# oooolga/Ctrl-V

Hardware: AMD Instinct MI355X
Metric: denoising steps/sec, SVD+ControlNet 25f 576x1024 (higher is better)
Workload: dtype bf16; 1 GPU; box2video: ControlNet + UNet forward, CFG batch 2, 25 frames, latent 72x128, 25-step Karras Euler schedule, random-init SVD-XT weights; clips_per_gpu=1, parallelism=clip-shard x1, hip_graph=True

## Files before the change

### ctrlv_amd/_lib.py

```python
import ctypes
import os
import threading

_HERE = os.path.dirname(os.path.abspath(__file__))
LIB_PATH = os.path.join(_HERE, "lib", "libctrlv_hip.so")
LIB_PATH_F16 = os.path.join(_HERE, "lib", "libctrlv_hip_f16.so")

c_void_p, c_int, c_float, c_size_t = ctypes.c_void_p, ctypes.c_int32, ctypes.c_float, ctypes.c_size_t


class GemmDesc(ctypes.Structure):
    _fields_ = [
        ("A", c_void_p), ("A2", c_void_p), ("W", c_void_p), ("out", c_void_p),
        ("bias", c_void_p), ("R1", c_void_p), ("R2", c_void_p), ("V", c_void_p),
        ("M", c_int), ("N", c_int), ("Cin", c_int), ("taps", c_int),
        ("lda", c_int), ("lda2", c_int), ("c_split", c_int),
        ("mode", c_int),
        ("H", c_int), ("Wd", c_int), ("Ho", c_int), ("Wo", c_int), ("stride", c_int), ("up", c_int),
        ("F", c_int), ("S", c_int),
        ("ldo", c_int), ("n_store", c_int),
        ("ldr1", c_int), ("ldr2", c_int),
        ("s_acc", c_float), ("s1", c_float), ("s2", c_float),
        ("vmode", c_int), ("vdiv", c_int), ("vmod", c_int), ("vS", c_int), ("ldv", c_int),
        ("act", c_int), ("geglu", c_int), ("out_f32", c_int), ("tile", c_int),
# ... 85 lines not shown
        ("latents", c_void_p), ("sigmas", ctypes.POINTER(c_float)), ("timesteps", ctypes.POINTER(c_float)),
        ("fps", c_int), ("motion_bucket_id", c_int),
        ("min_guidance", c_float), ("max_guidance", c_float), ("conditioning_scale", c_float), ("decode_chunk", c_int),
        ("clip_mean", c_float * 3), ("clip_std", c_float * 3),
        ("out_latents", c_void_p), ("out_frames", c_void_p), ("out_frames_u8", c_void_p),
    ]


SIGNATURES = {
    "ctrlv_abi_version": (c_int, []),
    "ctrlv_elem_dtype": (c_int, []),
    "ctrlv_build_id": (c_int, [ctypes.c_char_p, c_size_t]),
    "ctrlv_last_error": (c_int, [ctypes.c_char_p, c_size_t]),
    "ctrlv_gemm": (c_int, [ctypes.POINTER(GemmDesc), c_void_p]),
    "ctrlv_gemm_gn_partials_serves": (c_int, [ctypes.POINTER(GemmDesc)]),
    "ctrlv_gemm_splitk_ws_bytes": (c_size_t, [ctypes.POINTER(GemmDesc)]),
    "ctrlv_gemm_up_phase_serves": (c_int, [ctypes.POINTER(GemmDesc)]),
    "ctrlv_pack_up_phase_weight": (c_int, [c_void_p, c_int, c_int, c_int, c_void_p, c_void_p]),
    "ctrlv_groupnorm_from_partials": (c_int, [c_void_p, c_int, c_int, c_int, c_int, c_float, c_void_p, c_void_p, c_void_p,
                                              c_int, c_void_p, c_void_p]),
    "ctrlv_groupnorm_from_partials_split": (c_int, [c_void_p, c_void_p, c_int, c_int, c_int, c_int, c_float, c_void_p, c_void_p, c_void_p,
                                              c_int, c_void_p, c_void_p]),
    "ctrlv_groupnorm_chunks": (c_int, [c_int, c_int, c_int, c_int]),
    "ctrlv_groupnorm_stats_split": (c_int, [c_void_p, c_void_p, c_void_p, c_void_p, c_int, c_int, c_int, c_int, c_int, c_float,
                                            c_void_p, c_void_p]),
    "ctrlv_groupnorm_apply_split": (c_int, [c_void_p, c_void_p, c_void_p, c_void_p, c_int, c_int, c_int, c_int, c_int, c_void_p,
                                            c_void_p, c_void_p, c_int, c_void_p, c_void_p]),
    "ctrlv_layernorm_split": (c_int, [c_void_p, c_void_p, c_int, c_int, c_void_p, c_void_p, c_float, c_void_p, c_int, c_int,
                                      c_int, c_void_p, c_void_p]),
    "ctrlv_axpby_split": (c_int, [c_void_p, c_void_p, c_void_p, c_float, c_float, c_void_p, c_void_p, c_size_t, c_void_p]),
    "ctrlv_plan_set_trunk_mode": (c_int, [c_void_p, c_int]),
    "ctrlv_plan_set_ff_precision": (c_int, [c_void_p, c_int]),
    "ctrlv_groupnorm_stats": (c_int, [c_void_p, c_void_p, c_int, c_int, c_int, c_int, c_int, c_float, c_void_p,
                                      c_void_p]),
    "ctrlv_groupnorm_apply": (c_int, [c_void_p, c_void_p, c_int, c_int, c_int, c_int, c_int, c_void_p, c_void_p,
                                      c_void_p, c_int, c_void_p, c_void_p]),
    "ctrlv_layernorm": (c_int, [c_void_p, c_int, c_int, c_void_p, c_void_p, c_float, c_void_p, c_int, c_int, c_int,
                                c_void_p, c_void_p]),
    "ctrlv_softmax_rows": (c_int, [c_void_p, c_int, c_int, ctypes.c_long, c_void_p, ctypes.c_long, c_void_p]),
    "ctrlv_softmax_rows_bwd": (c_int, [c_void_p, ctypes.c_long, c_void_p, ctypes.c_long, c_int, c_int, c_float, c_void_p,
                                       ctypes.c_long, c_void_p]),
    "ctrlv_ff_fused_w1f_bytes": (c_int, []),
    "ctrlv_ff_fused_pack": (c_int, [c_void_p, c_void_p, c_void_p, c_void_p, c_void_p, c_void_p]),
    "ctrlv_ff_fused_serves": (c_int, [ctypes.POINTER(GemmDesc), c_int]),
    "ctrlv_ff_fused": (c_int, [c_void_p, c_int, c_void_p, c_void_p, ctypes.POINTER(GemmDesc), c_void_p]),
    "ctrlv_ff_fused_ln": (c_int, [c_void_p, c_int, c_void_p, c_void_p, c_float, c_void_p, c_int, c_int, c_int, c_void_p,
# ... 210 lines not shown
```

### ctrlv_amd/csrc/abi.hip

```cpp
#include <stdarg.h>
#include <stdlib.h>

#include <mutex>

#include "common.h"

#ifndef CTRLV_BUILD_ID
#define CTRLV_BUILD_ID "unstamped"
#endif

static thread_local char g_err[512] = "";
void ctrlv_set_error(const char* fmt, ...) {
  va_list ap;
  va_start(ap, fmt);
  vsnprintf(g_err, sizeof(g_err), fmt, ap);
  va_end(ap);
}

const ctrlv_debug_t& ctrlv_debug() {
  static const ctrlv_debug_t dbg = [] {
    auto env = [](const char* name, int dflt) { const char* e = getenv(name); return e ? atoi(e) : dflt; };
    ctrlv_debug_t d;
    d.w16 = env("CTRLV_W16", 1);
    d.splitk = env("CTRLV_SPLITK", 1);
    d.force_tile = env("CTRLV_GEMM_FORCE_TILE", 0);
    d.conv_halo = env("CTRLV_CONV_HALO", 1);
    d.gn_fused = env("CTRLV_GN_FUSED", 1);
    d.gn_cross = env("CTRLV_GN_CROSS", 1);
    d.gn_rev = env("CTRLV_GN_REV", 1);
    d.gn_rows = env("CTRLV_GN_ROWS", 256);
    if (d.gn_rows < 32 || d.gn_rows > 1024) d.gn_rows = 256;
    d.ln_rows = env("CTRLV_LN_ROWS", 1);
    d.ff_fused = env("CTRLV_FF_FUSED", 1);
    d.ff_ln = env("CTRLV_FF_LN", 0);
    d.pp_balanced = env("CTRLV_PP_BALANCED", 1);
    d.pp_cgrp = env("CTRLV_PP_CGRP", 0);
    d.attn_rows = env("CTRLV_ATTN_ROWS", 0);
    d.temporal_fused = env("CTRLV_TEMPORAL_FUSED", 1);
    d.wgrad_pp = env("CTRLV_WGRAD_PP", 1);
    d.wgrad_slabs = env("CTRLV_WGRAD_SLABS", 0);
    d.up_phase = env("CTRLV_UP_PHASE", 1);
    return d;
  }();
  return dbg;
}

int ctrlv_current_device() {
  int dev = 0;
  if (hipGetDevice(&dev) != hipSuccess || dev < 0 || dev >= CTRLV_MAX_DEVICES) dev = 0;
  return dev;
}

int ctrlv_num_cu(int dev) {
  static int cu[CTRLV_MAX_DEVICES] = {};
  static std::mutex mu;
// ... 33 lines not shown
```

### ctrlv_amd/csrc/common.h

```cpp
#pragma once
#include <hip/hip_runtime.h>
#include <stdint.h>
#include <stdio.h>
#include <string.h>

#include "../../include/ctrlv_hip.h"

#ifdef CTRLV_ELEM_F16
typedef _Float16 el_native_t;
#define CTRLV_ELEM_DTYPE 1
#define CTRLV_MFMA_32x32x16_ASM "v_mfma_f32_32x32x16_f16"
#else
typedef __bf16 el_native_t;
#define CTRLV_ELEM_DTYPE 2
#define CTRLV_MFMA_32x32x16_ASM "v_mfma_f32_32x32x16_bf16"
#endif
typedef __attribute__((ext_vector_type(8))) el_native_t elx8;
typedef __attribute__((ext_vector_type(4))) el_native_t elx4;
typedef __attribute__((ext_vector_type(2))) el_native_t elx2;
typedef __attribute__((ext_vector_type(16))) float f32x16;
typedef __attribute__((ext_vector_type(4))) float f32x4;
typedef __attribute__((ext_vector_type(4))) short s16x4;
typedef uint16_t el_t;
typedef uint16_t bf16_t;
// ... 227 lines not shown
  extern "C" int ctrlv_debug_clock_##unit(unsigned long long* out2, int reset) {                                   \
    if (hipDeviceSynchronize() != hipSuccess) return -3;                                                           \
    if (out2 && hipMemcpyFromSymbol(out2, HIP_SYMBOL(g_ctrlv_clock), 16) != hipSuccess) return -3;                 \
    const unsigned long long z[2] = {0, 0};                                                                        \
    if (reset && hipMemcpyToSymbol(HIP_SYMBOL(g_ctrlv_clock), z, 16) != hipSuccess) return -3;                     \
    return 0;                                                                                                      \
  }
#else
#define CTRLV_CLOCK_BEGIN()
#define CTRLV_CLOCK_END()
#define CTRLV_CLOCK_READER(unit)
#endif

struct ctrlv_debug_t {
  int w16;
  int splitk;
  int force_tile;
  int conv_halo;
  int gn_fused;
  int gn_cross;
  int gn_rev;
  int gn_rows;
  int ln_rows;
  int ff_fused;
  int ff_ln;
  int pp_balanced;
  int pp_cgrp;
  int attn_rows;
  int temporal_fused;
  int wgrad_pp;
  int wgrad_slabs;
  int up_phase;
};
const ctrlv_debug_t& ctrlv_debug();
void ctrlv_set_error(const char* fmt, ...);
#define CTRLV_MAX_DEVICES 64
int ctrlv_current_device();
int ctrlv_num_cu(int dev);
size_t ctrlv_gemm_tokens_counter_bytes(int M, int N, int K);
const ctrlv_model_config* ctrlv_plan_info(const ctrlv_plan* p, int* device, int* loaded);
const ctrlv_clip_config* ctrlv_clip_plan_info(const ctrlv_clip_plan* p, int* device, int* loaded);
const ctrlv_vae_config* ctrlv_vae_plan_info(const ctrlv_vae_plan* p, int* device, int* loaded);
#define CTRLV_CHECK_ARG(cond, ...)                  \
  do {                                              \
    if (!(cond)) {                                  \
      ctrlv_set_error(__VA_ARGS__);                 \
// ... 39 lines not shown
```

### ctrlv_amd/csrc/norm.hip

```cpp
#include <stdlib.h>

#include "common.h"

namespace {

struct GnShape {
  int n_img, S, C, imgs_per_stat, c_split, n_chunks, rows_per_chunk, CV, RPP;
  int rev_stats, rev_apply;
};

__device__ __forceinline__ uint4 gn_load(const el_t* x, const el_t* x2, int c_split, int C, long row, int c0) {
  if (x2 != nullptr && c0 >= c_split) return *(const uint4*)(x2 + row * (C - c_split) + (c0 - c_split));
  const int ld = x2 != nullptr ? c_split : C;
  return *(const uint4*)(x + row * ld + c0);
}
struct GnLo { const lo_t* x; const lo_t* x2; };
__device__ __forceinline__ const lo_t* gn_lo_plane(const GnLo& lo, const el_t* x2, int c_split, int C, int c0, int* ld, int* first) {
  if (x2 != nullptr && c0 >= c_split) { *ld = C - c_split; *first = c_split; return lo.x2; }
  *ld = x2 != nullptr ? c_split : C; *first = 0;
  return lo.x;
}

template <bool SPLIT>
__global__ void gn_stats_kernel(const el_t* __restrict__ x, const el_t* __restrict__ x2, GnLo lo, GnShape s,
// ... 158 lines not shown
  for (; r < r1; r += s.RPP) apply_row(gn_load(x, x2, s.c_split, s.C, (long)n * s.S + r, c0), (long)n * s.S + r);
}

int gn_shape(int n_img, int S, int C, int imgs_per_stat, int c_split, bool has_x2, GnShape* s) {
  CTRLV_CHECK_SHAPE(n_img > 0 && S > 0 && C > 0 && C % 32 == 0 && C % 8 == 0 && C <= 8192,
                    "groupnorm: C=%d must be a multiple of 32 (and of 8), <= 8192", C);
  CTRLV_CHECK_SHAPE(imgs_per_stat > 0 && n_img % imgs_per_stat == 0, "groupnorm: n_img %% imgs_per_stat != 0");
  if (has_x2) CTRLV_CHECK_SHAPE(c_split > 0 && c_split < C && c_split % 8 == 0, "groupnorm: bad c_split %d", c_split);
  s->n_img = n_img; s->S = S; s->C = C; s->imgs_per_stat = imgs_per_stat; s->c_split = c_split;
  s->CV = C / 8;
  s->RPP = s->CV >= 256 ? 1 : 256 / s->CV;
  {
    const int rev = ctrlv_debug().gn_rev;
    s->rev_stats = rev & 1; s->rev_apply = (rev >> 1) & 1;
  }
  {
    const int rpc_big = ctrlv_debug().gn_rows;
    s->rows_per_chunk = S >= 4096 ? rpc_big : (S >= 1024 ? 64 : 32);
  }
  if ((S + s->rows_per_chunk - 1) / s->rows_per_chunk > 256) s->rows_per_chunk = (((S + 255) / 256) + 255) / 256 * 256;
  if (s->rows_per_chunk > S) s->rows_per_chunk = S;
  s->n_chunks = (S + s->rows_per_chunk - 1) / s->rows_per_chunk;
  return CTRLV_OK;
}

template <int NV>
__global__ __launch_bounds__(256) void ln_kernel(const el_t* __restrict__ x, const lo_t* __restrict__ xlo, int M, int C,
                                                 const float* __restrict__ gamma, const float* __restrict__ beta,
                                                 float eps, const float* __restrict__ V, int vdiv, int vmod, int ldv,
                                                 el_t* __restrict__ y) {
  const int lane = threadIdx.x & 63, wid = threadIdx.x >> 6;
  const int CV = C >> 3;
  float g[NV][8], b[NV][8];
#pragma unroll
  for (int k = 0; k < NV; ++k) {
    const int cv = lane + k * 64;
    if (cv < CV) {
#pragma unroll
      for (int e = 0; e < 8; ++e) { g[k][e] = gamma[cv * 8 + e]; b[k][e] = beta[cv * 8 + e]; }
    }
  }
  const float inv_c = 1.0f / (float)C;
  const long step = (long)gridDim.x * 4;
  long m = (long)blockIdx.x * 4 + wid;
  uint4 nxt[NV];
#pragma unroll
// ... 297 lines not shown
  CTRLV_CHECK_ARG(x && partials && gamma && beta && y, "groupnorm_from_partials: null pointer");
  CTRLV_CHECK_SHAPE(S > 0 && S % 64 == 0, "groupnorm_from_partials: S=%d must be a multiple of 64", S);
  GnShape s;
  int rc = gn_shape(n_img, S, C, imgs_per_stat, 0, false, &s);
  if (rc < 0) return rc;
  GnShape sp = s;
  sp.rows_per_chunk = 64;
  sp.n_chunks = S / 64;
  float* stats = partials + (size_t)n_img * sp.n_chunks * 64;
  hipLaunchKernelGGL(gn_finalize_kernel, dim3(n_img / imgs_per_stat, 32 / kFinGroups), dim3(1024), 0, (hipStream_t)stream, sp,
                     partials, eps, stats);
  CTRLV_LAUNCH_CHECK();
  const int nt = s.CV * s.RPP;
  if (x_lo)
    hipLaunchKernelGGL(gn_apply_kernel<true>, dim3(s.n_chunks, n_img), dim3(nt), 0, (hipStream_t)stream, (const el_t*)x,
                       (const el_t*)nullptr, GnLo{(const lo_t*)x_lo, nullptr}, s, stats, gamma, beta, silu, (el_t*)y);
  else
    hipLaunchKernelGGL(gn_apply_kernel<false>, dim3(s.n_chunks, n_img), dim3(nt), 0, (hipStream_t)stream, (const el_t*)x,
                       (const el_t*)nullptr, GnLo{nullptr, nullptr}, s, stats, gamma, beta, silu, (el_t*)y);
  CTRLV_LAUNCH_CHECK();
  return CTRLV_OK;
}

extern "C" int ctrlv_layernorm(const void* x, int M, int C, const float* gamma, const float* beta, float eps,
                               const float* V, int vdiv, int vmod, int ldv, void* y, ctrlv_stream_t stream) {
  return ctrlv_layernorm_split(x, nullptr, M, C, gamma, beta, eps, V, vdiv, vmod, ldv, y, stream);
}
extern "C" int ctrlv_layernorm_split(const void* x, const void* x_lo, int M, int C, const float* gamma, const float* beta,
                                     float eps, const float* V, int vdiv, int vmod, int ldv, void* y, ctrlv_stream_t stream) {
  CTRLV_CHECK_ARG(x && gamma && beta && y, "layernorm: null pointer");
  CTRLV_CHECK_SHAPE(M > 0 && C > 0 && C % 8 == 0 && C <= 2048, "layernorm: C=%d must be a multiple of 8, <= 2048", C);
  if (V) CTRLV_CHECK_ARG(vdiv > 0 && vmod > 0 && ldv >= C, "layernorm: bad row-vector table");
  const int nv = (C / 8 + 63) / 64;
  hipStream_t st = (hipStream_t)stream;
  const int rows_path = ctrlv_debug().ln_rows;
  const int lpr = C / 40;
  if (rows_path && C % 40 == 0 && (lpr == 8 || lpr == 16 || lpr == 32) && (!V || (ldv % 4 == 0 && ((uintptr_t)V & 15) == 0))) {
    const int lg = lpr == 8 ? 3 : (lpr == 16 ? 4 : 5), rpb = 4 * (64 >> lg);
    long nb = ((long)M + rpb - 1) / rpb;
    if (nb > 256 * 8) nb = 256 * 8;
    if (x_lo)
      hipLaunchKernelGGL((ln_rows_kernel<5, true>), dim3((unsigned)nb), dim3(256), 2 * C * sizeof(float), st, (const el_t*)x,
                         (const lo_t*)x_lo, M, C, lg, gamma, beta, eps, V, vdiv, vmod, ldv, (el_t*)y);
    else
      hipLaunchKernelGGL((ln_rows_kernel<5, false>), dim3((unsigned)nb), dim3(256), 2 * C * sizeof(float), st, (const el_t*)x,
                         (const lo_t*)nullptr, M, C, lg, gamma, beta, eps, V, vdiv, vmod, ldv, (el_t*)y);
// ... 19 lines not shown
```

### ctrlv_amd/csrc/plan.hip

```cpp
#include <math.h>

#include <string>
#include <vector>

#include "weight_loader.h"

namespace {

using ctrlv_load::WeightLoader;
using Linear = ctrlv_load::PackedLinear;
using Norm = ctrlv_load::NormParams;

__global__ void arange_kernel(float* dst, int n) {
  const int i = blockIdx.x * blockDim.x + threadIdx.x;
  if (i < n) dst[i] = (float)i;
}
__global__ void expand_f32_kernel(const float* __restrict__ src, int n_src, float* __restrict__ dst, int n) {
  const int i = blockIdx.x * blockDim.x + threadIdx.x;
  if (i < n) dst[i] = src[n_src == 1 ? 0 : i];
}

struct ResBlock {
  int cin = 0, cout = 0;
  float eps = 1e-6f;
// ... 294 lines not shown
           (d.R1 ? (double)d.M * n_out * 2 : 0) + (d.R2 ? (double)d.M * n_out * 2 : 0) +
           ((d.R1_lo ? 1 : 0) + (d.R2_lo ? 1 : 0) + (d.out_lo ? 1 : 0)) * (double)d.M * n_out;
}
inline void set_r1(ctrlv_gemm_desc& d, const Trk& t, int ld) { d.R1 = t.hi; d.R1_lo = t.lo; d.ldr1 = ld; }
inline void set_r2(ctrlv_gemm_desc& d, const Trk& t, int ld) { d.R2 = t.hi; d.R2_lo = t.lo; d.ldr2 = ld; }
inline void set_out(ctrlv_gemm_desc& d, const Trk& t) { d.out = t.hi; d.out_lo = t.lo; }

int gemm(Ctx& c, const ctrlv_gemm_desc& d0) {
  ctrlv_gemm_desc d = d0;
  const size_t mk = c.mark();
  const size_t ws = ctrlv_gemm_splitk_ws_bytes(&d);
  if (ws) d.splitk_ws = c.alloc(ws);
  int rc = CTRLV_OK;
  if (!c.dry) {
    if (c.overflow) { ctrlv_set_error("plan forward: workspace too small (need >= %zu bytes)", c.peak); return CTRLV_E_BAD_ARG; }
    int fam; double fl, by;
    gemm_work(d, &fam, &fl, &by);
    ProfScope ps(c, fam, fl, by, d.M, d.N, (d.mode == 1 && d.up == 2 ? 4 : d.taps) * d.Cin, (d.geglu ? 1 : 0) | ((d.R1 ? 1 : 0) + (d.R2 ? 1 : 0)) << 1 | d.vmode << 3);
    rc = ctrlv_gemm(&d, c.st);
  }
  c.release(mk);
  return rc;
}
int groupnorm(Ctx& c, const Trk& x, const Trk& x2, int c_split, int n_img, int S, int C, int ips, const Norm& nm,
              float eps, int silu, el_t* y) {
  const int chunks = ctrlv_groupnorm_chunks(n_img, S, C, ips);
  if (chunks < 0) return chunks;
  const size_t m = c.mark();
  float* part = (float*)c.alloc(((size_t)n_img * chunks + n_img / ips) * 64 * 4);
  int rc = CTRLV_OK;
  if (!c.dry) {
    if (c.overflow) { ctrlv_set_error("plan forward: workspace too small (need >= %zu bytes)", c.peak); return CTRLV_E_BAD_ARG; }
    ProfScope ps(c, CTRLV_FAM_GROUPNORM, 0.0, 2.0 * 2 * n_img * (double)S * C, n_img * S, C);
    rc = ctrlv_groupnorm_stats_split(x.hi, x.lo, x2.hi, x2.lo, c_split, n_img, S, C, ips, eps, part, c.st);
    if (rc == CTRLV_OK)
      rc = ctrlv_groupnorm_apply_split(x.hi, x.lo, x2.hi, x2.lo, c_split, n_img, S, C, ips, part, nm.g, nm.b, silu, y, c.st);
  }
  c.release(m);
  return rc;
}
int gemm_groupnorm(Ctx& c, ctrlv_gemm_desc d, int n_img, int S, int C, int ips, const Norm& nm, float eps, int silu, el_t* y) {
  const Trk dout{(el_t*)d.out, (lo_t*)d.out_lo};
  if (S % 64 != 0) {
    CTRLV_TRY(gemm(c, d));
    return groupnorm(c, dout, Trk{}, 0, n_img, S, C, ips, nm, eps, silu, y);
  }
  const size_t m = c.mark();
  float* part = (float*)c.alloc(((size_t)n_img * (S / 64) + n_img / ips) * 64 * 4);
  int rc = CTRLV_OK;
  if (!c.dry && ctrlv_gemm_gn_partials_serves(&d)) {
    d.gn_partials = part;
    rc = gemm(c, d);
    if (rc == CTRLV_OK) {
      ProfScope ps(c, CTRLV_FAM_GROUPNORM, 0.0, 2.0 * 2 * n_img * (double)S * C, n_img * S, C, 1);
      rc = ctrlv_groupnorm_from_partials_split(d.out, d.out_lo, n_img, S, C, ips, eps, part, nm.g, nm.b, silu, y, c.st);
    }
// ... 887 lines not shown
```

### ctrlv_amd/models/blocks.py

```python
import math
import os

import torch
from torch import nn

from .. import ops, packing
from ..lora import merged_weight


class FwdCtx:

    def __init__(self, ws, B, F, temb, xattn, time_context_order):
        self.ws, self.B, self.F = ws, B, F
        self.temb = temb
        self.xattn = xattn
        self.quirk = time_context_order == "sb"
        self.gn_part = None
        self.gn_cross = None
        self.gn_cross_valid = False
        self.trace = None


def _sigmoid(x):
    return 1.0 / (1.0 + math.exp(-x))
# ... 153 lines not shown


def _ln_ff(ws, xraw, ln, t, ffp, ubox, out, C, ln_V=None, ln_vdiv=1, ln_vmod=1 << 30, rows_per_image=0, **epi):
    if _FF_FUSED and _FF_LN and len(ffp) == 6 and _lo(xraw) is None and ops.ff_fused_serves(xraw, out, **_trk_epi(epi, out)):
        ops.ff_fused(xraw, ffp[4], ffp[5], out, bias=ffp[3], ln=(ln[0], ln[1], 1e-5), ln_V=ln_V, ln_vdiv=ln_vdiv,
                     ln_vmod=ln_vmod, **_trk_epi(epi, out))
        return
    if getattr(ws, "ff_f8", False) and _lo(xraw) is None and _ff_f8_route(ws, xraw, ln, ffp, ubox, out, C, ln_V, ln_vdiv, ln_vmod, epi):
        return
    if ln_V is not None:
        ops.layernorm(xraw, ln[0], ln[1], 1e-5, t, V=ln_V, vdiv=ln_vdiv, vmod=ln_vmod, x_lo=_lo(xraw))
    else:
        ops.layernorm(xraw, ln[0], ln[1], 1e-5, t, x_lo=_lo(xraw))
    _ff_pair(ws, t, ffp, ubox, out, C, rows_per_image=rows_per_image, **epi)


def _gn_scratch(ctx, n_img, S, C, ips):
    need = ops.groupnorm_scratch_floats(n_img, S, C, ips)
    if ctx.gn_part is None or ctx.gn_part.numel() < need:
        ctx.gn_part = torch.empty(max(need, 1 << 18), dtype=torch.float32, device=ctx.ws.device)
    return ctx.gn_part


def _gemm_groupnorm(ctx, A, W, out, gkw, n_img, S, C, ips, gamma, beta, eps, y):
    gkw = _trk_epi(gkw, out)
    if S % 64 == 0 and ops.gemm_gn_partials_serves(A, W, out, **gkw):
        need = ops.groupnorm_fused_scratch_floats(n_img, S, ips)
        if ctx.gn_part is None or ctx.gn_part.numel() < need:
            ctx.gn_part = torch.empty(max(need, 1 << 18), dtype=torch.float32, device=ctx.ws.device)
        ops.gemm(A, W, out, gn_partials=ctx.gn_part, **gkw)
        ops.groupnorm_from_partials(out, n_img, S, C, ips, gamma, beta, eps, True, y, ctx.gn_part, x_lo=_lo(out))
    else:
        ops.gemm(A, W, out, **gkw)
        ops.groupnorm(out, None, n_img, S, C, ips, gamma, beta, eps, True, y, _gn_scratch(ctx, n_img, S, C, ips),
                      x_lo=_lo(out))


class SpatioTemporalResBlock(nn.Module):
    def __init__(self, in_channels, out_channels, temb_channels, eps=1e-6):
        super().__init__()
        self.cin, self.cout, self.eps = in_channels, out_channels, eps
        self.spatial_res_block = _ResnetBlock2D(in_channels, out_channels, temb_channels, eps)
        self.temporal_res_block = _TemporalResnetBlock(out_channels, temb_channels, eps)
        self.time_mixer = _AlphaBlender(0.5)
        self.temb_off = None
        self._pk = None

    def temb_projections(self):
        return [self.spatial_res_block.time_emb_proj, self.temporal_res_block.time_emb_proj]

    def pack(self):
        s, t = self.spatial_res_block, self.temporal_res_block
        pk = dict(
            g1=_f32(s.norm1.weight), b1=_f32(s.norm1.bias), w1=packing.pack_conv3x3(s.conv1.weight),
            cb1=_f32(s.conv1.bias),
            g2=_f32(s.norm2.weight), b2=_f32(s.norm2.bias), w2=packing.pack_conv3x3(s.conv2.weight),
            cb2=_f32(s.conv2.bias),
            tg1=_f32(t.norm1.weight), tb1=_f32(t.norm1.bias), tw1=packing.pack_conv_temporal(t.conv1.weight),
            tcb1=_f32(t.conv1.bias),
            tg2=_f32(t.norm2.weight), tb2=_f32(t.norm2.bias), tw2=packing.pack_conv_temporal(t.conv2.weight),
            tcb2=_f32(t.conv2.bias),
            alpha=_sigmoid(float(self.time_mixer.mix_factor.detach().float().cpu())),
        )
        if s.conv_shortcut is not None:
            pk["wsc"] = packing.pack_linear(s.conv_shortcut.weight)
            pk["bsc"] = _f32(s.conv_shortcut.bias)
        self._pk = pk

    def run(self, ctx, x, H, W, x2=None, feeds_norm=False):
        pk, ws = self._pk, ctx.ws
        B, F = ctx.B, ctx.F
        N, S = B * F, H * W
        M = N * S
        cin, cout = self.cin, self.cout
        out = ws.trunk((M, cout))
        mk = ws.mark()
        part = _gn_scratch(ctx, N, S, max(cin, cout), 1)
        xn = ws.alloc((M, cin))
        ops.groupnorm(x, x2, N, S, cin, 1, pk["g1"], pk["b1"], self.eps, True, xn, part, x_lo=_lo(x), x2_lo=_lo(x2))
        h = ws.alloc((M, cout))
        vs = ctx.temb[:, self.temb_off[0]:]
        hn = ws.alloc((M, cout))
        _gemm_groupnorm(ctx, xn, pk["w1"], h, dict(N=cout, cin=cin, taps=9, mode=1, conv=(H, W, H, W, 1, 0), bias=pk["cb1"],
                                                   V=vs, vmode=1, vdiv=F * S),
                        N, S, cout, 1, pk["g2"], pk["b2"], self.eps, hn)
        if "wsc" in pk:
            res = ws.trunk((M, cout))
            ops.gemm(x, pk["wsc"], res, N=cout, cin=cin, A2=x2, c_split=x.shape[1] if x2 is not None else 0,
                     bias=pk["bsc"], out_lo=_lo(res))
        else:
            res = x
        xs = ws.trunk((M, cout))
        _gemm_groupnorm(ctx, hn, pk["w2"], xs, dict(N=cout, cin=cout, taps=9, mode=1, conv=(H, W, H, W, 1, 0), bias=pk["cb2"],
                                                    R1=res),
                        N, S, cout, F, pk["tg1"], pk["tb1"], self.eps, hn)
        vt = ctx.temb[:, self.temb_off[1]:]
        _gemm_groupnorm(ctx, hn, pk["tw1"], h, dict(N=cout, cin=cout, taps=3, mode=2, temporal=(F, S), bias=pk["tcb1"],
                                                    V=vt, vmode=1, vdiv=F * S),
                        N, S, cout, F, pk["tg2"], pk["tb2"], self.eps, hn)
        kw2 = _trk_epi(dict(N=cout, cin=cout, taps=3, mode=2, temporal=(F, S), bias=pk["tcb2"], s_acc=1.0 - pk["alpha"], R1=xs),
                       out)
        ctx.gn_cross_valid = False
# ... 79 lines not shown
            kp = pk["tpe"][0].shape[1]
            te = torch.zeros(F, kp, dtype=el, device=device)
            if kp == C:
                ops.timestep_embedding(t, C, te)
            else:
                tmp = torch.empty(F, C, dtype=el, device=device)
                ops.timestep_embedding(t, C, tmp)
                te[:, :C] = tmp
            h = torch.empty(F, 4 * C, dtype=el, device=device)
            ops.gemm(te, pk["tpe"][0], h, N=4 * C, cin=kp, bias=pk["tpe"][1], act=1)
            e = torch.empty(F, C, dtype=torch.float32, device=device)
            ops.gemm(h, pk["tpe"][2], e, N=C, cin=4 * C, bias=pk["tpe"][3], out_f32=True)
            self._frame_emb[F] = e
        return self._frame_emb[F]

    def run(self, ctx, x, H, W):
        pk, ws = self._pk, ctx.ws
        B, F, C = ctx.B, ctx.F, self.C
        N, S = B * F, H * W
        M = N * S
        emb = self.frame_embedding(F, x.device)
        out = ws.trunk((M, C))
        mk = ws.mark()
        part = _gn_scratch(ctx, N, S, C, 1)
        t = ws.alloc((M, C))
        if ctx.gn_cross_valid:
            ctx.gn_cross_valid = False
            ops.groupnorm_from_partials(x, N, S, C, 1, pk["gn"][0], pk["gn"][1], 1e-6, False, t, ctx.gn_cross, x_lo=_lo(x))
        else:
            ops.groupnorm(x, None, N, S, C, 1, pk["gn"][0], pk["gn"][1], 1e-6, False, t, part, x_lo=_lo(x))
        h0 = ws.trunk((M, C))
        ops.gemm(t, pk["pin"][0], h0, N=C, cin=C, bias=pk["pin"][1], out_lo=_lo(h0))
        ops.layernorm(h0, pk["s_ln1"][0], pk["s_ln1"][1], 1e-5, t, x_lo=_lo(h0))
        qkv = ws.alloc((M, 3 * C))
        ops.gemm(t, pk["s_qkv"], qkv, N=3 * C, cin=C, n_scale2=C, s_acc2=ops.Q_PRESCALE)
        a = ws.alloc((M, C))
        ops.attention_spatial(qkv, a, N, S, C, prescaled=True)
        h1 = ws.trunk((M, C))
        xs_vec = ctx.xattn[:, self.xattn_off[0]:]
        ops.gemm(a, pk["s_o"][0], h1, N=C, cin=C, bias=pk["s_o"][1], **_trk_epi(dict(R1=h0, V=xs_vec, vmode=1, vdiv=F * S), h1))
        u = [None]
        h2 = h0
        _ln_ff(ws, h1, pk["s_ln3"], t, pk["s_ff"], u, h2, C, rows_per_image=S, R1=h1)
        g0 = h1
        _ln_ff(ws, h2, pk["t_lnin"], t, pk["t_ffin"], u, g0, C, ln_V=emb, ln_vdiv=S, ln_vmod=F, rows_per_image=S, R1=h2, V=emb, vmode=1, vdiv=S,
               vmod=F)
        g1 = ws.trunk((M, C))
        xt_vec = ctx.xattn[:, self.xattn_off[1]:]
        vkw = dict(vmode=2, vdiv=F * S, vS=S, vmod=B) if (ctx.quirk and B > 1) else dict(vmode=1, vdiv=F * S)
        fkw = _trk_epi(dict(bias=pk["t_o"][1], R1=g0, V=xt_vec, ln=(pk["t_ln1"][0], pk["t_ln1"][1], 1e-5), **vkw), g1)
        if _TEMPORAL_FUSED and ops.temporal_fused_serves(g0, pk["t_wf"], g1, B, F, S, **fkw):
            ops.temporal_fused(g0, pk["t_wf"], g1, B, F, S, **fkw)
        else:
# ... 171 lines not shown
```

### ctrlv_amd/models/unet_spatio_temporal_condition.py

```python
from dataclasses import dataclass
from typing import Optional, Tuple, Union

import torch
from torch import nn

from .. import lora, ops, packing
from .blocks import CrossAttnUpBlockSpatioTemporal, UpBlockSpatioTemporal, _f32, _gn_scratch, _lo
from .encoder import SpatioTemporalEncoderBase, _tup


@dataclass
class UNetSpatioTemporalConditionOutput:
    sample: torch.Tensor = None

    def __getitem__(self, i):
        return (self.sample,)[i]


class UNetSpatioTemporalConditionModel(SpatioTemporalEncoderBase):
    _class_name = "UNetSpatioTemporalConditionModel"
    _supports_gradient_checkpointing = True

    def __init__(
        self,
        sample_size: Optional[int] = None,
        in_channels: int = 8,
        out_channels: int = 4,
        down_block_types: Tuple[str] = ("CrossAttnDownBlockSpatioTemporal", "CrossAttnDownBlockSpatioTemporal",
                                        "CrossAttnDownBlockSpatioTemporal", "DownBlockSpatioTemporal"),
        up_block_types: Tuple[str] = ("UpBlockSpatioTemporal", "CrossAttnUpBlockSpatioTemporal",
# ... 143 lines not shown
        x, H, W, taps = self._run_down_mid(ctx, x, h, w)
        if is_controlnet:
            if len(down_block_additional_residuals) != len(taps):
                raise ValueError(f"expected {len(taps)} down_block_additional_residuals, got "
                                 f"{len(down_block_additional_residuals)}")
            ev = getattr(self, "_residual_event", None)
            if ev is not None:
                torch.cuda.current_stream().wait_event(ev)
            mk = ws.mark()
            def add_res(t, r):
                rr = self._residual_rows(ws, r, t.shape[0], t.shape[1])
                if _lo(t) is not None:
                    ops.axpby_split(t, _lo(t), rr, 1.0, 1.0, t, _lo(t))
                else:
                    ops.axpby(t, rr, 1.0, 1.0, t)
            for (s, sh, sw), r in zip(taps, down_block_additional_residuals):
                add_res(s, r)
            add_res(x, mid_block_additional_residuals)
            ws.release(mk)
        skips = [t[0] for t in taps]
        for blk in self.up_blocks:
            x, H, W = blk.run(ctx, x, H, W, skips)
        M, c0 = x.shape
        part = _gn_scratch(ctx, N, H * W, c0, 1)
        xn = ws.alloc((M, c0))
        ops.groupnorm(x, None, N, H * W, c0, 1, pk["gno"][0], pk["gno"][1], 1e-5, True, xn, part, x_lo=_lo(x))
        co = self.config.out_channels
        co_p = (co + 3) // 4 * 4
        y = ws.alloc((M, co_p))
        ops.gemm(xn, pk["cout_w"], y, N=pk["cout_w"].shape[0], cin=c0, taps=9, mode=1, conv=(H, W, H, W, 1, 0),
                 bias=pk["cout_b"], n_store=co_p)
        out = torch.empty(N, co, H, W, dtype=sample.dtype, device=sample.device)
        ops.rows_to_nchw(y, out)
        out = out.reshape(B, F, co, H, W)
        if not return_dict:
            return (out,)
        return UNetSpatioTemporalConditionOutput(sample=out)
```

### ctrlv_amd/ops.py

```python
import ctypes

import torch

from . import _lib, profiler as _prof
from ._lib import GemmDesc, check

_DT = {torch.float32: 0, torch.float16: 1, torch.bfloat16: 2}


def _stream():
    return ctypes.c_void_p(torch.cuda.current_stream().cuda_stream)


def _p(t):
    return None if t is None else ctypes.c_void_p(t.data_ptr())


def _L(*tensors):
    els = {t.dtype for t in tensors if t is not None and t.dtype in (torch.float16, torch.bfloat16)}
    if len(els) > 1:
        raise ValueError("ctrlv_amd: one call mixes bf16 and fp16 element tensors (a library serves ONE element type)")
    return _lib.load(torch.float16 if torch.float16 in els else None)


# ... 346 lines not shown
        check(rc, "ctrlv_groupnorm_chunks")
    return rc


def groupnorm_scratch_floats(n_img, S, C, imgs_per_stat):
    return (n_img * groupnorm_chunks(n_img, S, C, imgs_per_stat) + n_img // imgs_per_stat) * 64


def groupnorm_fused_scratch_floats(n_img, S, imgs_per_stat):
    return (n_img * (S // 64) + n_img // imgs_per_stat) * 64


def groupnorm_from_partials(x, n_img, S, C, imgs_per_stat, gamma, beta, eps, silu, y, partials, x_lo=None):
    _need_gpu(x, "x")
    assert partials.numel() >= groupnorm_fused_scratch_floats(n_img, S, imgs_per_stat)
    ev = _prof.begin()
    check(_L(x).ctrlv_groupnorm_from_partials_split(_p(x), _p(x_lo), n_img, S, C, imgs_per_stat, eps, _p(partials), _p(gamma),
                                                    _p(beta), 1 if silu else 0, _p(y), _stream()),
          "ctrlv_groupnorm_from_partials")
    _prof.end(ev, "groupnorm", 0.0, 2.0 * 2 * n_img * S * C)
    return y


def groupnorm(x, x2, n_img, S, C, imgs_per_stat, gamma, beta, eps, silu, y, partials, x_lo=None, x2_lo=None):
    _need_gpu(x, "x")
    lib = _L(x)
    c_split = x.shape[1] if x2 is not None else 0
    st = _stream()
    ev = _prof.begin()
    check(lib.ctrlv_groupnorm_stats_split(_p(x), _p(x_lo), _p(x2), _p(x2_lo), c_split, n_img, S, C, imgs_per_stat, eps,
                                          _p(partials), st), "ctrlv_groupnorm_stats")
    check(lib.ctrlv_groupnorm_apply_split(_p(x), _p(x_lo), _p(x2), _p(x2_lo), c_split, n_img, S, C, imgs_per_stat,
                                          _p(partials), _p(gamma), _p(beta), 1 if silu else 0, _p(y), st),
          "ctrlv_groupnorm_apply")
    _prof.end(ev, "groupnorm", 0.0, 2.0 * 2 * n_img * S * C)
    return y


def layernorm(x, gamma, beta, eps, y, V=None, vdiv=1, vmod=1 << 30, x_lo=None):
    _need_gpu(x, "x")
    M, C = x.shape
    ev = _prof.begin()
    check(_L(x).ctrlv_layernorm_split(_p(x), _p(x_lo), M, C, _p(gamma), _p(beta), eps, _p(V), vdiv, vmod,
                                      V.stride(0) if V is not None else 0, _p(y), _stream()), "ctrlv_layernorm")
    _prof.end(ev, "layernorm", 0.0, 2.0 * 2 * M * C)
    return y
# ... 339 lines not shown
```

### include/ctrlv_hip.h

```cpp
#ifndef CTRLV_HIP_H
#define CTRLV_HIP_H

#include <stddef.h>
#include <stdint.h>

#ifdef __cplusplus
extern "C" {
#endif

typedef void* ctrlv_stream_t;

enum {
  CTRLV_OK = 0,
  CTRLV_E_BAD_ARG = -1,
  CTRLV_E_BAD_SHAPE = -2,
  CTRLV_E_HIP = -3,
  CTRLV_E_BAD_DTYPE = -4,
  CTRLV_E_WORKSPACE = -5,
};

int ctrlv_abi_version(void);
int ctrlv_elem_dtype(void);
int ctrlv_build_id(char* buf, size_t n);
int ctrlv_last_error(char* buf, size_t n);
// ... 37 lines not shown
int ctrlv_gemm(const ctrlv_gemm_desc* d, ctrlv_stream_t stream);
size_t ctrlv_gemm_splitk_ws_bytes(const ctrlv_gemm_desc* d);
int ctrlv_gemm_gn_partials_serves(const ctrlv_gemm_desc* d);
int ctrlv_gemm_up_phase_serves(const ctrlv_gemm_desc* d);
int ctrlv_pack_up_phase_weight(const void* w, int dtype, int N, int Cin, void* dst, ctrlv_stream_t stream);

int ctrlv_groupnorm_chunks(int n_img, int S, int C, int imgs_per_stat);
int ctrlv_groupnorm_stats(const void* x, const void* x2, int c_split, int n_img, int S, int C, int imgs_per_stat,
                          float eps, float* partials, ctrlv_stream_t stream);
int ctrlv_groupnorm_apply(const void* x, const void* x2, int c_split, int n_img, int S, int C, int imgs_per_stat,
                          const float* partials, const float* gamma, const float* beta, int silu, void* y,
                          ctrlv_stream_t stream);
int ctrlv_groupnorm_from_partials(const void* x, int n_img, int S, int C, int imgs_per_stat, float eps, float* partials,
                                  const float* gamma, const float* beta, int silu, void* y, ctrlv_stream_t stream);
int ctrlv_groupnorm_from_partials_split(const void* x, const void* x_lo, int n_img, int S, int C, int imgs_per_stat, float eps,
                                        float* partials, const float* gamma, const float* beta, int silu, void* y,
                                        ctrlv_stream_t stream);
int ctrlv_groupnorm_stats_split(const void* x, const void* x_lo, const void* x2, const void* x2_lo, int c_split, int n_img,
                                int S, int C, int imgs_per_stat, float eps, float* partials, ctrlv_stream_t stream);
int ctrlv_groupnorm_apply_split(const void* x, const void* x_lo, const void* x2, const void* x2_lo, int c_split, int n_img,
                                int S, int C, int imgs_per_stat, const float* partials, const float* gamma,
                                const float* beta, int silu, void* y, ctrlv_stream_t stream);

int ctrlv_layernorm(const void* x, int M, int C, const float* gamma, const float* beta, float eps,
                    const float* V, int vdiv, int vmod, int ldv, void* y, ctrlv_stream_t stream);
int ctrlv_layernorm_split(const void* x, const void* x_lo, int M, int C, const float* gamma, const float* beta, float eps,
                          const float* V, int vdiv, int vmod, int ldv, void* y, ctrlv_stream_t stream);

int ctrlv_ff_fused_w1f_bytes(void);
int ctrlv_ff_fused_pack(const void* w1_packed, const float* b1, const void* w2_packed, void* w1f, void* w2f,
                        ctrlv_stream_t stream);
int ctrlv_ff_fused(const void* x, int ldx, const void* w1f, const void* w2f, const ctrlv_gemm_desc* out_desc,
                   ctrlv_stream_t stream);
int ctrlv_ff_fused_ln(const void* x, int ldx, const float* ln_gamma, const float* ln_beta, float ln_eps,
                      const float* ln_V, int ln_vdiv, int ln_vmod, int ln_ldv, const void* w1f, const void* w2f,
                      const ctrlv_gemm_desc* out_desc, ctrlv_stream_t stream);
int ctrlv_ff_fused_serves(const ctrlv_gemm_desc* out_desc, int ldx);

int ctrlv_quant_rows_f8(const void* x, int M, int K, int ldx, const float* gamma, const float* beta, float eps,
                        const float* V, int vdiv, int vmod, int ldv, void* q, int ldq, float* scale, ctrlv_stream_t stream);
int ctrlv_gemm_f8(const ctrlv_gemm_desc* d, const float* a_scale, const float* w_scale, ctrlv_stream_t stream);
int ctrlv_gemm_f8_serves(const ctrlv_gemm_desc* d);

typedef struct ctrlv_temporal_fused_desc {
  const void* x; int32_t ldx;
  const void* wf;
// ... 255 lines not shown
```

Baseline: 4.667 steps/s.

## Add register-resident one-pass GroupNorm kernel for small spatial sizes

Adds a GroupNorm kernel that loads each group's slab into registers once, computes the mean (shifted by a pivot) and the variance with two in-block reductions, then normalizes and writes from registers in a single launch. It replaces the separate stats and apply kernels, and their second read of x, when S*imgs_per_stat fits in one block and no lo split is present. This mainly helps the low-resolution UNet/ControlNet stages. It trades fewer launches and less memory traffic for one block per group chunk, which can limit parallelism, and it is on by default via an env var.

```diff
diff --git a/ctrlv_amd/_lib.py b/ctrlv_amd/_lib.py
--- a/ctrlv_amd/_lib.py
+++ b/ctrlv_amd/_lib.py
@@ -131,6 +131,9 @@
     "ctrlv_groupnorm_from_partials_split": (c_int, [c_void_p, c_void_p, c_int, c_int, c_int, c_int, c_float, c_void_p, c_void_p, c_void_p,
                                               c_int, c_void_p, c_void_p]),
     "ctrlv_groupnorm_chunks": (c_int, [c_int, c_int, c_int, c_int]),
+    "ctrlv_groupnorm_onepass_serves": (c_int, [c_int, c_int, c_int, c_int, c_int]),
+    "ctrlv_groupnorm_onepass": (c_int, [c_void_p, c_void_p, c_int, c_int, c_int, c_int, c_int, c_float, c_void_p, c_void_p,
+                                        c_int, c_void_p, c_void_p, c_void_p]),
     "ctrlv_groupnorm_stats_split": (c_int, [c_void_p, c_void_p, c_void_p, c_void_p, c_int, c_int, c_int, c_int, c_int, c_float,
                                             c_void_p, c_void_p]),
     "ctrlv_groupnorm_apply_split": (c_int, [c_void_p, c_void_p, c_void_p, c_void_p, c_int, c_int, c_int, c_int, c_int, c_void_p,
diff --git a/ctrlv_amd/csrc/abi.hip b/ctrlv_amd/csrc/abi.hip
--- a/ctrlv_amd/csrc/abi.hip
+++ b/ctrlv_amd/csrc/abi.hip
@@ -31,6 +31,7 @@
     d.gn_rows = env("CTRLV_GN_ROWS", 256);
     if (d.gn_rows < 32 || d.gn_rows > 1024) d.gn_rows = 256;
     d.ln_rows = env("CTRLV_LN_ROWS", 1);
+    d.gn_onepass = env("CTRLV_GN_ONEPASS", 1);
     d.ff_fused = env("CTRLV_FF_FUSED", 1);
     d.ff_ln = env("CTRLV_FF_LN", 0);
     d.pp_balanced = env("CTRLV_PP_BALANCED", 1);
diff --git a/ctrlv_amd/csrc/common.h b/ctrlv_amd/csrc/common.h
--- a/ctrlv_amd/csrc/common.h
+++ b/ctrlv_amd/csrc/common.h
@@ -273,6 +273,7 @@
   int gn_rev;
   int gn_rows;
   int ln_rows;
+  int gn_onepass;
   int ff_fused;
   int ff_ln;
   int pp_balanced;
diff --git a/ctrlv_amd/csrc/norm.hip b/ctrlv_amd/csrc/norm.hip
--- a/ctrlv_amd/csrc/norm.hip
+++ b/ctrlv_amd/csrc/norm.hip
@@ -204,6 +204,202 @@
   if (s->rows_per_chunk > S) s->rows_per_chunk = S;
   s->n_chunks = (S + s->rows_per_chunk - 1) / s->rows_per_chunk;
   return CTRLV_OK;
+}
+
+struct GnOne { int C, c_split, cpg, BV, RPP, R; };
+constexpr int kOneMaxLoads = 24;
+
+template <int GB>
+__device__ __forceinline__ void gn_one_block_sum(float (&sg)[GB], float* red, int lane, int wid, int nw) {
+#pragma unroll
+  for (int g = 0; g < GB; ++g) {
+    sg[g] = wave_sum(sg[g]);
+    if (lane == 0) red[wid * GB + g] = sg[g];
+  }
+  __syncthreads();
+#pragma unroll
+  for (int g = 0; g < GB; ++g) {
+    float t = 0.f;
+    for (int w = 0; w < nw; ++w) t += red[w * GB + g];
+    sg[g] = t;
+  }
+}
+
+template <int NL, int GB>
+__global__ __launch_bounds__(1024) void gn_onepass_kernel(const el_t* __restrict__ x, const el_t* __restrict__ x2, GnOne s,
+                                                          float eps, const float* __restrict__ gamma,
+                                                          const float* __restrict__ beta, int silu, el_t* __restrict__ y,
+                                                          float* __restrict__ stats_out) {
+  __shared__ float red[2][16 * GB];
+  const int tid = threadIdx.x, lane = tid & 63, wid = tid >> 6, nw = (int)blockDim.x >> 6;
+  const int nblk = 32 / GB;
+  const int w = xcd_remap(blockIdx.x, gridDim.x);
+  const int stat = w / nblk, blk = w % nblk;
+  const int col = tid % s.BV, rsub = tid / s.BV;
+  const int cb = blk * s.BV * 8, c0 = cb + col * 8;
+  const long row0 = (long)stat * s.R;
+  const bool live = rsub < s.RPP;
+  const bool in2 = x2 != nullptr && c0 >= s.c_split;
+  const int ldx = in2 ? s.C - s.c_split : (x2 != nullptr ? s.c_split : s.C);
+  const el_t* px = (in2 ? x2 + (c0 - s.c_split) : x + c0) + (row0 + rsub) * ldx;
+  const long xstep = (long)s.RPP * ldx;
+  uint4 v[NL];
+#pragma unroll
+  for (int u = 0; u < NL; ++u) {
+    const int r = rsub + u * s.RPP;
+    v[u] = (live && r < s.R) ? *(const uint4*)(px + u * xstep) : make_uint4(0, 0, 0, 0);
+  }
+  float K;
+  {
+    float pf[8];
+    unpack_elx8(gn_load(x, x2, s.c_split, s.C, row0, cb), pf);
+    K = pf[0];
+  }
+  int gl[8];
+#pragma unroll
+  for (int e = 0; e < 8; ++e) gl[e] = GB == 1 ? 0 : (col * 8 + e) / s.cpg;
+  float sg[GB];
+  {
+    float ss[8];
+#pragma unroll
+    for (int e = 0; e < 8; ++e) ss[e] = 0.f;
+#pragma unroll
+    for (int u = 0; u < NL; ++u) {
+      if (live && rsub + u * s.RPP < s.R) {
+        float f[8];
+        unpack_elx8(v[u], f);
+#pragma unroll
+        for (int e = 0; e < 8; ++e) ss[GB == 1 ? 0 : e] += f[e] - K;
+      }
+    }
+#pragma unroll
+    for (int g = 0; g < GB; ++g) {
+      sg[g] = 0.f;
+#pragma unroll
+      for (int e = 0; e < 8; ++e) sg[g] += (GB == 1 || gl[e] == g) ? ss[e] : 0.f;
+    }
+  }
+  gn_one_block_sum<GB>(sg, red[0], lane, wid, nw);
+  const float cnt = (float)s.cpg * (float)s.R, inv_cnt = 1.0f / cnt;
+  float mean[GB], me[8];
+#pragma unroll
+  for (int g = 0; g < GB; ++g) mean[g] = K + sg[g] * inv_cnt;
+#pragma unroll
+  for (int e = 0; e < 8; ++e) {
+    me[e] = mean[0];
+#pragma unroll
+    for (int g = 1; g < GB; ++g) me[e] = gl[e] == g ? mean[g] : me[e];
+  }
+  {
+    float ss[8];
+#pragma unroll
+    for (int e = 0; e < 8; ++e) ss[e] = 0.f;
+#pragma unroll
+    for (int u = 0; u < NL; ++u) {
+      if (live && rsub + u * s.RPP < s.R) {
+        float f[8];
+        unpack_elx8(v[u], f);
+#pragma unroll
+        for (int e = 0; e < 8; ++e) { const float dl = f[e] - me[e]; ss[GB == 1 ? 0 : e] += dl * dl; }
+      }
+    }
+#pragma unroll
+    for (int g = 0; g < GB; ++g) {
+      sg[g] = 0.f;
+#pragma unroll
+      for (int e = 0; e < 8; ++e) sg[g] += (GB == 1 || gl[e] == g) ? ss[e] : 0.f;
+    }
+  }
+  gn_one_block_sum<GB>(sg, red[1], lane, wid, nw);
+  float rstd[GB];
+#pragma unroll
+  for (int g = 0; g < GB; ++g) {
+    rstd[g] = (float)(1.0 / sqrt((double)sg[g] / (double)cnt + (double)eps));
+    if (stats_out != nullptr && tid == g) {
+      stats_out[((long)stat * 32 + blk * GB + g) * 2] = mean[g];
+      stats_out[((long)stat * 32 + blk * GB + g) * 2 + 1] = rstd[g];
+    }
+  }
+  if (!live) return;
+  if (NL > 16) {
+    static_assert(NL <= 16 || GB == 1, "slabs deeper than 16 loads: one group per block");
+#pragma unroll
+    for (int h = 0; h < 2; ++h) {
+      const float4 g4 = *(const float4*)(gamma + c0 + 4 * h), b4 = *(const float4*)(beta + c0 + 4 * h);
+      const float gg[4] = {g4.x, g4.y, g4.z, g4.w}, bb[4] = {b4.x, b4.y, b4.z, b4.w};
+      float a[4], b[4];
+#pragma unroll
+      for (int e = 0; e < 4; ++e) {
+        a[e] = rstd[0] * gg[e];
+        b[e] = bb[e] - mean[0] * a[e];
+      }
+#pragma unroll
+      for (int u = 0; u < NL; ++u) {
+        const int r = rsub + u * s.RPP;
+        if (r < s.R) {
+          float f[4];
+          const uint32_t w0 = h ? v[u].z : v[u].x, w1 = h ? v[u].w : v[u].y;
+          f[0] = el_lo_f32(w0); f[1] = el_hi_f32(w0); f[2] = el_lo_f32(w1); f[3] = el_hi_f32(w1);
+#pragma unroll
+          for (int e = 0; e < 4; ++e) {
+            const float t = f[e] * a[e] + b[e];
+            f[e] = silu ? silu_f(t) : t;
+          }
+          *(uint2*)(y + (row0 + r) * s.C + c0 + 4 * h) = make_uint2(pack_elx2(f[0], f[1]), pack_elx2(f[2], f[3]));
+        }
+      }
+    }
+    return;
+  }
+  float a[8], b[8];
+  {
+    const float4 g0 = *(const float4*)(gamma + c0), g1 = *(const float4*)(gamma + c0 + 4);
+    const float4 b0 = *(const float4*)(beta + c0), b1 = *(const float4*)(beta + c0 + 4);
+    const float gg[8] = {g0.x, g0.y, g0.z, g0.w, g1.x, g1.y, g1.z, g1.w};
+    const float bb[8] = {b0.x, b0.y, b0.z, b0.w, b1.x, b1.y, b1.z, b1.w};
+#pragma unroll
+    for (int e = 0; e < 8; ++e) {
+      float rs = rstd[0];
+#pragma unroll
+      for (int g = 1; g < GB; ++g) rs = gl[e] == g ? rstd[g] : rs;
+      a[e] = rs * gg[e];
+      b[e] = bb[e] - me[e] * a[e];
+    }
+  }
+#pragma unroll
+  for (int u = 0; u < NL; ++u) {
+    const int r = rsub + u * s.RPP;
+    if (r < s.R) {
+      float f[8];
+      unpack_elx8(v[u], f);
+#pragma unroll
+      for (int e = 0; e < 8; ++e) {
+        const float t = f[e] * a[e] + b[e];
+        f[e] = silu ? silu_f(t) : t;
+      }
+      *(uint4*)(y + (row0 + r) * s.C + c0) = pack_elx8(f);
+    }
+  }
+}
+
+bool gn_one_plan(int S, int C, int imgs_per_stat, int c_split, GnOne* o, int* nl, int* gb, int* nt) {
+  if (S <= 0 || S > 1024 || C <= 0 || C % 32 != 0 || C > 8192 || imgs_per_stat <= 0) return false;
+  if (c_split != 0 && (c_split < 0 || c_split >= C || c_split % 8 != 0)) return false;
+  const int cpg = C / 32;
+  int g = 8;
+  while (cpg % g != 0) g >>= 1;
+  const int GB = 8 / g, BV = cpg / g;
+  const long R = (long)imgs_per_stat * S;
+  const int rpp_max = 1024 / BV;
+  if (rpp_max < 1) return false;
+  const long nl_min = (R + rpp_max - 1) / rpp_max;
+  if (nl_min > kOneMaxLoads) return false;
+  const int NL = nl_min <= 4 ? 4 : (nl_min <= 8 ? 8 : (nl_min <= 16 ? 16 : kOneMaxLoads));
+  if (NL > 8 && GB != 1) return false;
+  const int RPP = (int)((R + NL - 1) / NL);
+  o->C = C; o->c_split = c_split; o->cpg = cpg; o->BV = BV; o->RPP = RPP; o->R = (int)R;
+  *nl = NL; *gb = GB; *nt = (BV * RPP + 63) / 64 * 64;
+  return true;
 }
 
 template <int NV>
@@ -547,6 +743,46 @@
   return CTRLV_OK;
 }
 
+extern "C" int ctrlv_groupnorm_onepass_serves(int n_img, int S, int C, int imgs_per_stat, int c_split) {
+  GnOne o;
+  int nl, gb, nt;
+  return n_img > 0 && gn_one_plan(S, C, imgs_per_stat, c_split, &o, &nl, &gb, &nt) ? 1 : 0;
+}
+
+extern "C" int ctrlv_groupnorm_onepass(const void* x, const void* x2, int c_split, int n_img, int S, int C, int imgs_per_stat,
+                                       float eps, const float* gamma, const float* beta, int silu, void* y, float* stats_out,
+                                       ctrlv_stream_t stream) {
+  CTRLV_CHECK_ARG(x && gamma && beta && y, "groupnorm_onepass: null pointer");
+  CTRLV_CHECK_SHAPE(n_img > 0 && imgs_per_stat > 0 && n_img % imgs_per_stat == 0, "groupnorm_onepass: n_img %% imgs_per_stat != 0");
+  if (x2) CTRLV_CHECK_SHAPE(c_split > 0 && c_split < C && c_split % 8 == 0, "groupnorm_onepass: bad c_split %d", c_split);
+  GnOne o;
+  int nl = 0, gb = 0, nt = 0;
+  CTRLV_CHECK_SHAPE(gn_one_plan(S, C, imgs_per_stat, x2 ? c_split : 0, &o, &nl, &gb, &nt),
+                    "groupnorm_onepass: (S=%d, C=%d, imgs_per_stat=%d) is not served (ctrlv_groupnorm_onepass_serves)", S, C,
+                    imgs_per_stat);
+  const dim3 grid((32 / gb) * (n_img / imgs_per_stat));
+#define GN_ONE_LAUNCH(NL, GB)                                                                                              \
+  hipLaunchKernelGGL((gn_onepass_kernel<NL, GB>), grid, dim3(nt), 0, (hipStream_t)stream, (const el_t*)x, (const el_t*)x2, o, \
+                     eps, gamma, beta, silu, (el_t*)y, stats_out)
+#define GN_ONE_GB(NL)                                                                                                      \
+  switch (gb) {                                                                                                            \
+    case 1: GN_ONE_LAUNCH(NL, 1); break;                                                                                   \
+    case 2: GN_ONE_LAUNCH(NL, 2); break;                                                                                   \
+    case 4: GN_ONE_LAUNCH(NL, 4); break;                                                                                   \
+    default: GN_ONE_LAUNCH(NL, 8); break;                                                                                  \
+  }
+  switch (nl) {
+    case 4: GN_ONE_GB(4); break;
+    case 8: GN_ONE_GB(8); break;
+    case 16: GN_ONE_LAUNCH(16, 1); break;
+    default: GN_ONE_LAUNCH(kOneMaxLoads, 1); break;
+  }
+#undef GN_ONE_GB
+#undef GN_ONE_LAUNCH
+  CTRLV_LAUNCH_CHECK();
+  return CTRLV_OK;
+}
+
 extern "C" int ctrlv_layernorm(const void* x, int M, int C, const float* gamma, const float* beta, float eps,
                                const float* V, int vdiv, int vmod, int ldv, void* y, ctrlv_stream_t stream) {
   return ctrlv_layernorm_split(x, nullptr, M, C, gamma, beta, eps, V, vdiv, vmod, ldv, y, stream);
diff --git a/ctrlv_amd/csrc/plan.hip b/ctrlv_amd/csrc/plan.hip
--- a/ctrlv_amd/csrc/plan.hip
+++ b/ctrlv_amd/csrc/plan.hip
@@ -340,6 +340,9 @@
   c.release(mk);
   return rc;
 }
+inline bool gn_onepass(const Trk& x, const Trk& x2, int c_split, int n_img, int S, int C, int ips) {
+  return ctrlv_debug().gn_onepass && ips == 1 && !x.lo && !x2.lo && ctrlv_groupnorm_onepass_serves(n_img, S, C, ips, c_split);
+}
 int groupnorm(Ctx& c, const Trk& x, const Trk& x2, int c_split, int n_img, int S, int C, int ips, const Norm& nm,
               float eps, int silu, el_t* y) {
   const int chunks = ctrlv_groupnorm_chunks(n_img, S, C, ips);
@@ -350,6 +353,11 @@
   if (!c.dry) {
     if (c.overflow) { ctrlv_set_error("plan forward: workspace too small (need >= %zu bytes)", c.peak); return CTRLV_E_BAD_ARG; }
     ProfScope ps(c, CTRLV_FAM_GROUPNORM, 0.0, 2.0 * 2 * n_img * (double)S * C, n_img * S, C);
+    if (gn_onepass(x, x2, c_split, n_img, S, C, ips)) {
+      rc = ctrlv_groupnorm_onepass(x.hi, x2.hi, c_split, n_img, S, C, ips, eps, nm.g, nm.b, silu, y, nullptr, c.st);
+      c.release(m);
+      return rc;
+    }
     rc = ctrlv_groupnorm_stats_split(x.hi, x.lo, x2.hi, x2.lo, c_split, n_img, S, C, ips, eps, part, c.st);
     if (rc == CTRLV_OK)
       rc = ctrlv_groupnorm_apply_split(x.hi, x.lo, x2.hi, x2.lo, c_split, n_img, S, C, ips, part, nm.g, nm.b, silu, y, c.st);
diff --git a/ctrlv_amd/models/blocks.py b/ctrlv_amd/models/blocks.py
--- a/ctrlv_amd/models/blocks.py
+++ b/ctrlv_amd/models/blocks.py
@@ -199,6 +199,18 @@
     return ctx.gn_part
 
 
+def _gn_onepass(x, x2, n_img, S, C, ips):
+    return ops.GN_ONEPASS and ips == 1 and ops.groupnorm_onepass_serves(n_img, S, C, ips, x.shape[1] if x2 is not None else 0,
+                                                           has_lo=_lo(x) is not None or _lo(x2) is not None)
+
+
+def groupnorm(ctx, x, x2, n_img, S, C, ips, gamma, beta, eps, silu, y):
+    if _gn_onepass(x, x2, n_img, S, C, ips):
+        return ops.groupnorm_onepass(x, x2, n_img, S, C, ips, gamma, beta, eps, silu, y)
+    return ops.groupnorm(x, x2, n_img, S, C, ips, gamma, beta, eps, silu, y, _gn_scratch(ctx, n_img, S, C, ips),
+                         x_lo=_lo(x), x2_lo=_lo(x2))
+
+
 def _gemm_groupnorm(ctx, A, W, out, gkw, n_img, S, C, ips, gamma, beta, eps, y):
     gkw = _trk_epi(gkw, out)
     if S % 64 == 0 and ops.gemm_gn_partials_serves(A, W, out, **gkw):
@@ -209,8 +221,7 @@
         ops.groupnorm_from_partials(out, n_img, S, C, ips, gamma, beta, eps, True, y, ctx.gn_part, x_lo=_lo(out))
     else:
         ops.gemm(A, W, out, **gkw)
-        ops.groupnorm(out, None, n_img, S, C, ips, gamma, beta, eps, True, y, _gn_scratch(ctx, n_img, S, C, ips),
-                      x_lo=_lo(out))
+        groupnorm(ctx, out, None, n_img, S, C, ips, gamma, beta, eps, True, y)
 
 
 class SpatioTemporalResBlock(nn.Module):
@@ -252,9 +263,9 @@
         cin, cout = self.cin, self.cout
         out = ws.trunk((M, cout))
         mk = ws.mark()
-        part = _gn_scratch(ctx, N, S, max(cin, cout), 1)
+        _gn_scratch(ctx, N, S, max(cin, cout), 1)
         xn = ws.alloc((M, cin))
-        ops.groupnorm(x, x2, N, S, cin, 1, pk["g1"], pk["b1"], self.eps, True, xn, part, x_lo=_lo(x), x2_lo=_lo(x2))
+        groupnorm(ctx, x, x2, N, S, cin, 1, pk["g1"], pk["b1"], self.eps, True, xn)
         h = ws.alloc((M, cout))
         vs = ctx.temb[:, self.temb_off[0]:]
         hn = ws.alloc((M, cout))
@@ -380,13 +391,13 @@
         emb = self.frame_embedding(F, x.device)
         out = ws.trunk((M, C))
         mk = ws.mark()
-        part = _gn_scratch(ctx, N, S, C, 1)
+        _gn_scratch(ctx, N, S, C, 1)
         t = ws.alloc((M, C))
         if ctx.gn_cross_valid:
             ctx.gn_cross_valid = False
             ops.groupnorm_from_partials(x, N, S, C, 1, pk["gn"][0], pk["gn"][1], 1e-6, False, t, ctx.gn_cross, x_lo=_lo(x))
         else:
-            ops.groupnorm(x, None, N, S, C, 1, pk["gn"][0], pk["gn"][1], 1e-6, False, t, part, x_lo=_lo(x))
+            groupnorm(ctx, x, None, N, S, C, 1, pk["gn"][0], pk["gn"][1], 1e-6, False, t)
         h0 = ws.trunk((M, C))
         ops.gemm(t, pk["pin"][0], h0, N=C, cin=C, bias=pk["pin"][1], out_lo=_lo(h0))
         ops.layernorm(h0, pk["s_ln1"][0], pk["s_ln1"][1], 1e-5, t, x_lo=_lo(h0))
diff --git a/ctrlv_amd/models/unet_spatio_temporal_condition.py b/ctrlv_amd/models/unet_spatio_temporal_condition.py
--- a/ctrlv_amd/models/unet_spatio_temporal_condition.py
+++ b/ctrlv_amd/models/unet_spatio_temporal_condition.py
@@ -5,7 +5,7 @@
 from torch import nn
 
 from .. import lora, ops, packing
-from .blocks import CrossAttnUpBlockSpatioTemporal, UpBlockSpatioTemporal, _f32, _gn_scratch, _lo
+from .blocks import CrossAttnUpBlockSpatioTemporal, UpBlockSpatioTemporal, _f32, _lo, groupnorm as _groupnorm
 from .encoder import SpatioTemporalEncoderBase, _tup
 
 
@@ -195,9 +195,8 @@
         for blk in self.up_blocks:
             x, H, W = blk.run(ctx, x, H, W, skips)
         M, c0 = x.shape
-        part = _gn_scratch(ctx, N, H * W, c0, 1)
         xn = ws.alloc((M, c0))
-        ops.groupnorm(x, None, N, H * W, c0, 1, pk["gno"][0], pk["gno"][1], 1e-5, True, xn, part, x_lo=_lo(x))
+        _groupnorm(ctx, x, None, N, H * W, c0, 1, pk["gno"][0], pk["gno"][1], 1e-5, True, xn)
         co = self.config.out_channels
         co_p = (co + 3) // 4 * 4
         y = ws.alloc((M, co_p))
diff --git a/ctrlv_amd/ops.py b/ctrlv_amd/ops.py
--- a/ctrlv_amd/ops.py
+++ b/ctrlv_amd/ops.py
@@ -1,4 +1,5 @@
 import ctypes
+import os
 
 import torch
 
@@ -392,6 +393,25 @@
     return y
 
 
+GN_ONEPASS = os.environ.get("CTRLV_GN_ONEPASS", "1") not in ("", "0")
+
+
+def groupnorm_onepass_serves(n_img, S, C, imgs_per_stat, c_split=0, has_lo=False):
+    if has_lo:
+        return False
+    return bool(_lib.load().ctrlv_groupnorm_onepass_serves(n_img, S, C, imgs_per_stat, c_split))
+
+
+def groupnorm_onepass(x, x2, n_img, S, C, imgs_per_stat, gamma, beta, eps, silu, y, stats_out=None):
+    _need_gpu(x, "x")
+    c_split = x.shape[1] if x2 is not None else 0
+    ev = _prof.begin()
+    check(_L(x).ctrlv_groupnorm_onepass(_p(x), _p(x2), c_split, n_img, S, C, imgs_per_stat, eps, _p(gamma), _p(beta),
+                                        1 if silu else 0, _p(y), _p(stats_out), _stream()), "ctrlv_groupnorm_onepass")
+    _prof.end(ev, "groupnorm", 0.0, 2.0 * 2 * n_img * S * C)
+    return y
+
+
 def groupnorm(x, x2, n_img, S, C, imgs_per_stat, gamma, beta, eps, silu, y, partials, x_lo=None, x2_lo=None):
     _need_gpu(x, "x")
     lib = _L(x)
diff --git a/include/ctrlv_hip.h b/include/ctrlv_hip.h
--- a/include/ctrlv_hip.h
+++ b/include/ctrlv_hip.h
@@ -83,6 +83,10 @@
                                 int S, int C, int imgs_per_stat, const float* partials, const float* gamma,
                                 const float* beta, int silu, void* y, ctrlv_stream_t stream);
 
+int ctrlv_groupnorm_onepass_serves(int n_img, int S, int C, int imgs_per_stat, int c_split);
+int ctrlv_groupnorm_onepass(const void* x, const void* x2, int c_split, int n_img, int S, int C, int imgs_per_stat, float eps,
+                            const float* gamma, const float* beta, int silu, void* y, float* stats_out, ctrlv_stream_t stream);
+
 int ctrlv_layernorm(const void* x, int M, int C, const float* gamma, const float* beta, float eps,
                     const float* V, int vdiv, int vmod, int ldv, void* y, ctrlv_stream_t stream);
 int ctrlv_layernorm_split(const void* x, const void* x_lo, int M, int C, const float* gamma, const float* beta, float eps,
```

After: 4.677 steps/s (median of 6 runs). Within noise of the previous version (+0.2%).
